# ZJU-FAST-Lab/uneven_planner

Measured on AMD Instinct MI355X. Metric: MINCO traj-opts/sec (batch), higher is better.
Workload: dtype f64

## Files before the change

### include/uneven_hip.h

```cpp
#ifndef UNEVEN_HIP_H
#define UNEVEN_HIP_H

#include <stdint.h>

#ifdef __cplusplus
extern "C" {
#endif

typedef struct uph_map uph_map;
typedef struct uph_ctx uph_ctx;
typedef struct uph_kino uph_kino;

#define UPH_OK 0
#define UPH_ERR_INVALID (-1)
#define UPH_ERR_HIP (-2)
#define UPH_ERR_NO_DEVICE (-3)
#define UPH_ERR_LIMIT (-4)
#define UPH_ERR_NO_CACHE (-5)

#define UPH_RET_STOPPED 3
#define UPH_RET_UNSUPPORTED 4

#define UPH_RET_LEFT_TILE 5
#define UPH_TILE_MARGIN 2.0
// ... 181 lines not shown
int uph_traj_states(uph_ctx* c, int32_t n, const int32_t* traj, const double* t, double* out10);
#define UPH_REFINE_AT_END 7
int uph_refine_upload(uph_ctx* src, uph_ctx* dst, int32_t B, const int32_t* src_traj, const double* t_switch, double* switch_states ,
                      int32_t* status, int32_t* traj_of, int32_t* n_inner_xy, int32_t* n_inner_yaw);
int uph_plan_staged(uph_ctx* c, int32_t cap_xy, int32_t cap_yaw, double* init_xy, double* end_xy, double* init_yaw, double* end_yaw, double* inner_xy,
                    double* inner_yaw, int32_t* n_inner_xy, int32_t* n_inner_yaw, double* total_time);

int uph_ctx_create(uph_map* m, const uph_opt_params* p, uph_ctx** out);
void uph_ctx_destroy(uph_ctx* c);
int uph_ctx_set_lanes(uph_ctx* c, int32_t lanes);
int uph_ctx_set_xcd_locality(uph_ctx* c, int32_t group);
int uph_ctx_set_wps(uph_ctx* c, int32_t wps);
int uph_ctx_set_sample_precision(uph_ctx* c, int32_t bits);
int uph_ctx_set_rho(uph_ctx* c, double rho);
int uph_ctx_get_rho(uph_ctx* c, double* rho);

int uph_ctx_set_trace(uph_ctx* c, int32_t cap);
int uph_ctx_get_trace(uph_ctx* c, double* out);

int uph_optimize_batch(uph_ctx* c, int32_t B, const uph_problem* probs, uph_result* results);
int uph_optimize_batch_multi(uph_ctx* const* ctxs, int32_t n_gpus, int32_t B, const uph_problem* probs, uph_result* results);
int uph_multi_batch_plan(int32_t n_gpus, int32_t B, const uph_problem* probs, int32_t* share_of, double* predicted_cost);
int uph_batch_count(const uph_ctx* c);
int uph_batch_origin(const uph_ctx* c, int32_t* idx);
int uph_batch_upload(uph_ctx* c, int32_t B, const uph_problem* probs);
int uph_batch_solve(uph_ctx* c);
int uph_batch_solve_async(uph_ctx* c);
int uph_batch_wait(uph_ctx* c);
int uph_batch_download(uph_ctx* c, uph_result* results);
int uph_batch_stats(uph_ctx* c, double* kernel_ms, int64_t* evals, int64_t* sample_evals, int64_t* lbfgs_iters, int64_t* hist_bytes);

int uph_batch_prepare_ms(uph_ctx* c, double* ms);

int uph_batch_cycles(uph_ctx* c, long long* out);

int uph_eval_batch(uph_ctx* c, const double* x_packed, double* f, double* grad_packed, int32_t repeat);
int uph_penalty_batch(uph_ctx* c, int32_t repeat, int32_t store_residuals, double* cost, double* gdcxy_packed, double* gdcyaw_packed, double* gdT2);
int uph_init_scaling_batch(uph_ctx* c);
int uph_microbench_batch(uph_ctx* c, int32_t reps);
int uph_batch_set_state(uph_ctx* c, const double* lambda, const double* mu, const double* scale_cx, const double* scale_fx, const double* rho);
int uph_batch_set_x(uph_ctx* c, const double* x_packed);
int uph_batch_alm_passes(uph_ctx* c, int32_t max_passes);
int uph_batch_set_lbfgs_state(uph_ctx* c, const double* g, const double* d, const double* pf, const double* lm_s, const double* lm_y, const double* lm_ys, const double* scal5);
int uph_batch_lbfgs_resume(uph_ctx* c, int32_t budget, int32_t finish_pass);
int uph_batch_get_lbfgs_state(uph_ctx* c, double* g, double* d, double* pf, double* lm_s, double* lm_y, double* lm_ys, double* scal8);
// ... 45 lines not shown
```

### uneven_planner_amd/_lib.py

```python
import ctypes as C
import os

_HERE = os.path.dirname(os.path.abspath(__file__))
LIB_PATH = os.environ.get("UNEVENHIP_LIB") or os.path.join(_HERE, "libunevenhip.so")


class MapParams(C.Structure):
    _fields_ = [("iter_num", C.c_int32), ("map_size_x", C.c_double), ("map_size_y", C.c_double),
                ("ellipsoid_x", C.c_double), ("ellipsoid_y", C.c_double), ("ellipsoid_z", C.c_double),
                ("xy_resolution", C.c_double), ("yaw_resolution", C.c_double), ("min_cnormal", C.c_double),
                ("max_rho", C.c_double), ("gravity", C.c_double)]


class OptParams(C.Structure):
    _fields_ = [("rho_T", C.c_double), ("rho_ter", C.c_double), ("max_vel", C.c_double), ("max_acc_lon", C.c_double),
                ("max_acc_lat", C.c_double), ("max_kap", C.c_double), ("min_cxi", C.c_double), ("max_sig", C.c_double),
                ("use_scaling", C.c_int32), ("rho", C.c_double), ("beta", C.c_double), ("gamma", C.c_double),
                ("epsilon_con", C.c_double), ("max_iter", C.c_double), ("g_epsilon", C.c_double),
                ("min_step", C.c_double), ("inner_max_iter", C.c_double), ("delta", C.c_double),
                ("mem_size", C.c_int32), ("past", C.c_int32), ("int_K", C.c_int32)]


class ManagerParams(C.Structure):
    _fields_ = [("piece_len", C.c_double), ("mean_vel", C.c_double), ("init_time_times", C.c_double), ("yaw_piece_times", C.c_double),
# ... 85 lines not shown
    "uph_frontend_query": (C.c_int, [_VP, DP, _I32, DP, C.POINTER(C.c_int32), C.POINTER(C.c_int32)]),
    "uph_terrain_pose_query": (C.c_int, [_VP, DP, _I32, DP]),
    "uph_frontend_query_ms": (C.c_int, [_VP, DP]),
    "uph_map_filter_cloud": (_I64, [C.POINTER(C.c_float), _I64, C.POINTER(C.c_float), _I64]),
    "uph_map_build_stats": (C.c_int, [_VP, DP, C.POINTER(_I64), C.POINTER(_I64)]),
    "uph_map_build_stages": (C.c_int, [_VP, DP]),
    "uph_map_built_cloud": (_I64, [_VP, C.POINTER(C.c_float), _I64]),
    "uph_ctx_create": (C.c_int, [_VP, C.POINTER(OptParams), C.POINTER(_VP)]),
    "uph_ctx_destroy": (None, [_VP]),
    "uph_ctx_set_lanes": (C.c_int, [_VP, _I32]),
    "uph_ctx_set_wps": (C.c_int, [_VP, _I32]),
    "uph_ctx_set_xcd_locality": (C.c_int, [_VP, _I32]),
    "uph_ctx_set_sample_precision": (C.c_int, [_VP, _I32]),
    "uph_ctx_set_rho": (C.c_int, [_VP, C.c_double]),
    "uph_ctx_get_rho": (C.c_int, [_VP, DP]),
    "uph_ctx_set_trace": (C.c_int, [_VP, _I32]),
    "uph_ctx_get_trace": (C.c_int, [_VP, DP]),
    "uph_optimize_batch": (C.c_int, [_VP, _I32, C.POINTER(Problem), C.POINTER(Result)]),
    "uph_batch_upload": (C.c_int, [_VP, _I32, C.POINTER(Problem)]),
    "uph_batch_solve": (C.c_int, [_VP]),
    "uph_batch_solve_async": (C.c_int, [_VP]),
    "uph_batch_wait": (C.c_int, [_VP]),
    "uph_batch_download": (C.c_int, [_VP, C.POINTER(Result)]),
    "uph_batch_stats": (C.c_int, [_VP, DP, C.POINTER(_I64), C.POINTER(_I64), C.POINTER(_I64), C.POINTER(_I64)]),
    "uph_batch_prepare_ms": (C.c_int, [_VP, DP]),
    "uph_batch_cycles": (C.c_int, [_VP, C.POINTER(C.c_longlong)]),
    "uph_build_id": (C.c_char_p, []),
    "uph_eval_batch": (C.c_int, [_VP, DP, DP, DP, _I32]),
    "uph_penalty_batch": (C.c_int, [_VP, _I32, _I32, DP, DP, DP, DP]),
    "uph_init_scaling_batch": (C.c_int, [_VP]),
    "uph_microbench_batch": (C.c_int, [_VP, _I32]),
    "uph_batch_set_state": (C.c_int, [_VP, DP, DP, DP, DP, DP]),
    "uph_report_batch": (C.c_int, [_VP, DP]),
    "uph_rollout_sizes": (C.c_int, [_I32, C.POINTER(_I32), DP, C.POINTER(_I32), DP, C.c_double, _I32, C.POINTER(_I64)]),
    "uph_rollout_plan": (C.c_int, [_VP, C.c_double, _I32, C.POINTER(_I64)]),
    "uph_rollout_batch": (C.c_int, [_VP, C.c_double, _I32, _I32, _I32, _I32, DP]),
    "uph_rollout_batch_dev": (C.c_int, [_VP, C.c_double, _I32, _I32, _I32, _I32, _VP]),
    "uph_batch_set_x": (C.c_int, [_VP, DP]),
    "uph_batch_alm_passes": (C.c_int, [_VP, _I32]),
    "uph_batch_set_lbfgs_state": (C.c_int, [_VP, DP, DP, DP, DP, DP, DP, DP]),
# ... 105 lines not shown
```

### uneven_planner_amd/alm_traj_opt.py

```python
import ctypes as C

import numpy as np

from . import _lib

HILL_OPT_PARAMS = dict(rho_T=100000.0, rho_ter=10.0, max_vel=0.5, max_acc_lon=5.0, max_acc_lat=10.0, max_kap=2.1,
                       min_cxi=0.8, max_sig=0.05, use_scaling=True, rho=1.0, beta=1000.0, gamma=1.0,
                       epsilon_con=0.001, max_iter=10.0, g_epsilon=1.0e-3, min_step=1.0e-32, inner_max_iter=10000.0,
                       delta=1.0e-4, mem_size=256, past=3, int_K=16)
_INT_FIELDS = ("use_scaling", "mem_size", "past", "int_K")


def pack_problems(probs, int_K=16, with_sizes=False):
    arr = (_lib.Problem * len(probs))()
    keep, sizes = [], []
    for i, pr in enumerate(probs):
        ixy = np.ascontiguousarray(np.asarray(pr["inner_xy"], dtype=np.float64).T)
        iyw = np.ascontiguousarray(pr["inner_yaw"], dtype=np.float64)
        keep += [ixy, iyw]
        a = arr[i]
        a.n_inner_xy, a.n_inner_yaw = ixy.shape[0], iyw.shape[0]
        a.init_xy[:] = np.asarray(pr["init_xy"], dtype=np.float64).T.ravel().tolist()
        a.end_xy[:] = np.asarray(pr["end_xy"], dtype=np.float64).T.ravel().tolist()
        a.init_yaw[:] = np.asarray(pr["init_yaw"], dtype=np.float64).ravel().tolist()
# ... 370 lines not shown
    def set_lanes(self, lanes):
        _lib.check(self.L.uph_ctx_set_lanes(self.h, int(lanes)), "uph_ctx_set_lanes")

    def set_xcd_locality(self, group):
        _lib.check(self.L.uph_ctx_set_xcd_locality(self.h, int(group)), "uph_ctx_set_xcd_locality")

    def set_wps(self, wps):
        _lib.check(self.L.uph_ctx_set_wps(self.h, int(wps)), "uph_ctx_set_wps")

    def set_sample_precision(self, bits):
        _lib.check(self.L.uph_ctx_set_sample_precision(self.h, int(bits)), "uph_ctx_set_sample_precision")

    def set_rho(self, rho):
        _lib.check(self.L.uph_ctx_set_rho(self.h, float(rho)), "uph_ctx_set_rho")

    def get_rho(self):
        r = C.c_double(0)
        _lib.check(self.L.uph_ctx_get_rho(self.h, C.byref(r)), "uph_ctx_get_rho")
        return r.value

    def _make_problems(self, probs):
        arr, keep, self._sizes = pack_problems(probs, int(self.int_K), with_sizes=True)
        return arr, keep

    def upload(self, probs):
        arr, keep = self._make_problems(probs)
        self._B = 0
        _lib.check(self.L.uph_batch_upload(self.h, len(probs), arr), "uph_batch_upload")
        self._B = len(probs)
        self._trace_cap_up = getattr(self, "_trace_cap", 0)
# ... 1 lines not shown
    def solve(self):
        _lib.check(self.L.uph_batch_solve(self.h), "uph_batch_solve")

    def solve_async(self):
        _lib.check(self.L.uph_batch_solve_async(self.h), "uph_batch_solve_async")

    def wait(self):
        _lib.check(self.L.uph_batch_wait(self.h), "uph_batch_wait")

    def stats(self):
        ms = C.c_double(0)
        v = [C.c_int64(0) for _ in range(4)]
        _lib.check(self.L.uph_batch_stats(self.h, C.byref(ms), *[C.byref(x) for x in v]), "uph_batch_stats")
        pm = C.c_double(0)
        _lib.check(self.L.uph_batch_prepare_ms(self.h, C.byref(pm)), "uph_batch_prepare_ms")
        return dict(kernel_ms=ms.value, prepare_ms=pm.value, evals=v[0].value, sample_evals=v[1].value, lbfgs_iters=v[2].value, hist_bytes=v[3].value)

    def cycles(self):
        out = np.zeros((max(0, self.L.uph_batch_count(self.h)), 16), dtype=np.int64)
        _lib.check(self.L.uph_batch_cycles(self.h, out.ctypes.data_as(C.POINTER(C.c_longlong))), "uph_batch_cycles")
        return out

    def origin(self):
        idx = np.zeros(max(0, self.L.uph_batch_count(self.h)), dtype=np.int32)
        _lib.check(self.L.uph_batch_origin(self.h, idx.ctypes.data_as(C.POINTER(C.c_int32))), "uph_batch_origin")
        return idx

    def download(self, full=True):
        res, bufs = self._result_array(self._sizes, full)
        _lib.check(self.L.uph_batch_download(self.h, res), "uph_batch_download")
        self._last = self._collect(res, bufs)
# ... 479 lines not shown
```

### uneven_planner_amd/csrc/solver_program.hpp

```cpp
#pragma once
#include "terrain_dev.hpp"
#include "trajectory_dev.hpp"
#include "uph_common.hpp"

namespace uph {

#ifndef UPH_GRID_FROM_MEM
#define UPH_GRID_FROM_MEM 1
#endif
#ifndef UPH_PHASE_MASK
#define UPH_PHASE_MASK 15
#endif
#ifndef UPH_SCALING_WB
#define UPH_SCALING_WB 8
#endif
#ifndef UPH_SC_XB
#define UPH_SC_XB 9
#endif
#ifndef UPH_SC_YB
#define UPH_SC_YB 14
#endif
#ifndef UPH_SC_WLO
#define UPH_SC_WLO 2
#endif
#ifndef UPH_SC_WHI
#define UPH_SC_WHI 3
#endif

template <class WG, class SR = double>
struct Solver {
    WG& wg;
    const GridDev& grid;
    const OptParams& P;
    const BatchDev& bd;
    const TrajDesc& td;
    int Nxy, Nyaw, n, S, K, mem, CH, CHP, recd;
    int CHS;
    int* rtag;
    double *x, *xp, *g, *gp, *d, *cxy, *cyaw, *Gxy, *Gyaw, *gamxy, *gamyaw, *bt, *rec, *wtab, *ttab, *pf, *hd;
    double *dual, *res, *scl, *hist;
    int hrow, hnp;
    const double *Wr_xy, *Wr_yaw;
    double rho, scale_fx, Txy, Tyaw, last_jerk, last_gd;
    long long hist_reads;
    long long cyc[16];
    long long t_last_eval_end;
    long long* sub_t = nullptr;
    int evals, bidx, trace_n;
    float inv_k1;
    double ec_irho, ec_step, ec_invK, ec_iTyaw, ec_omega, ec_omega_h;

    static constexpr int REC_FIELDS = 12;
    static UPH_HD size_t ldsDoubles(int Nxy, int Nyaw, int n, int CH, int mem, int K) {
        size_t recd = (size_t)REC_FIELDS * (CH + 1) + (CH + 1) / 2;
        const size_t nvec = 2 * (Nxy + 5) + (Nyaw + 5);
        const size_t knd = (size_t)knotBufDoubles(Nxy + 1, 4) + knotBufDoubles(Nyaw + 1, 2), adj = (size_t)knotBufDoubles(Nxy, 4) + knotBufDoubles(Nyaw, 2) + nvec;
        recd = recd < knd ? knd : recd;
        recd = recd < adj ? adj : recd;
        recd = recd < (size_t)mem ? (size_t)mem : recd;
        const size_t td_ = (size_t)Nxy + K + 2;
        return (size_t)5 * n + (nvec < td_ ? td_ : nvec) + 2 * (12 * Nxy + 6 * Nyaw) + recd + (size_t)6 * (K + 1) + THOMAS_DOUBLES + MAX_PAST + 8 + 18;
    }

    UPH_HD Solver(WG& w, const GridDev& gr, const OptParams& p, const BatchDev& b, int bi, double* lds)
        : wg(w), grid(gr), P(p), bd(b), td(b.desc[bi]) {
        bidx = bi;
        Nxy = td.Nxy; Nyaw = td.Nyaw; n = td.n; S = td.S; K = P.int_K; mem = P.mem_size;
        inv_k1 = 1.0f / (float)(K + 1);
        CH = wg.size(); CHP = CH + 1; recd = REC_FIELDS * CHP + (CH + 1) / 2;
        CHS = CH;
#if !defined(UPH_ALIGNED_CHUNKS) || UPH_ALIGNED_CHUNKS
        {
            const int ppc = CH / (K + 1);
            if (ppc >= 1 && (Nxy + ppc - 1) / ppc == (S + CH - 1) / CH) CHS = ppc * (K + 1);
        }
#endif
// ... 6 lines not shown
        q += nvec < Nxy + K + 2 ? Nxy + K + 2 : nvec;
        cxy = q; q += 12 * Nxy; cyaw = q; q += 6 * Nyaw;
        Gxy = q; q += 12 * Nxy; Gyaw = q; q += 6 * Nyaw;
        wtab = q; q += 6 * (K + 1);
        rec = q;
        {
            size_t rd = (size_t)recd;
            const size_t knd = (size_t)knotBufDoubles(Nxy + 1, 4) + knotBufDoubles(Nyaw + 1, 2), adj = (size_t)knotBufDoubles(Nxy, 4) + knotBufDoubles(Nyaw, 2) + nvec;
            rd = rd < knd ? knd : rd; rd = rd < adj ? adj : rd; rd = rd < (size_t)mem ? (size_t)mem : rd;
            q += rd;
        }
        rtag = (int*)(rec + (size_t)REC_FIELDS * CHP);
        ttab = q; q += THOMAS_DOUBLES;
        pf = q; q += MAX_PAST + 8;
        hd = q; q += 18;
        dual = bd.dual + 7 * td.off_s; res = bd.res + 7 * td.off_s; scl = bd.scl + 7 * td.off_s;
        hist = bd.hist + td.off_hist; hrow = histRowDoubles(n); hnp = 64 * histNQ(n);
        Wr_xy = bd.ops[td.op_xy].Wr; Wr_yaw = bd.ops[td.op_yaw].Wr;
        rho = 0; scale_fx = 1.0; Txy = Tyaw = 0; last_jerk = 0; hist_reads = 0; evals = 0; trace_n = 0;
        for (int q = 0; q < 16; q++) cyc[q] = 0;
        t_last_eval_end = 0;
        wg.pfor(18 + THOMAS_DOUBLES, [&](int t) {
            if (t < 18) hd[t] = t < 6 ? td.init_xy[t] : (t < 12 ? td.end_xy[t - 6] : (t < 15 ? td.init_yaw[t - 12] : td.end_yaw[t - 15]));
            else ttab[t - 18] = bd.thomas[t - 18];
        });
    }

    UPH_HD void tracePush(double v) {
        if (bd.trace != nullptr && trace_n < bd.trace_cap) {
            const int at = trace_n;
            wg.one([&]() { bd.trace[(size_t)bidx * bd.trace_cap + at] = v; });
        }
        trace_n++;
    }

    static UPH_HD int divSmall(int a, int b, float inv) {
        int q = (int)((float)a * inv);
// ... 584 lines not shown

    UPH_HD void evalConsts() {
        ec_irho = wg.bcast(1.0 / rho);
        ec_step = wg.bcast(Txy / K);
        ec_invK = wg.bcast(1.0 / K);
        ec_omega = wg.bcast(P.rho_ter * ec_step * scale_fx);
        ec_omega_h = wg.bcast(0.5 * P.rho_ter * ec_step * scale_fx);
    }

    UPH_HD void refreshResiduals() {
        UPH_MARK("refreshResiduals");
        wg.pfor(2, [&](int u) { fillTimes(u); });
        wg.pfor(S, [&](int s) { double dummy[3]; sampleEval<true>(s, 0, dummy); });
    }

    template <bool STEP>
    UPH_HD double eval(double* xin, double* gout, double st = 0.0) {
        evals++;
        long long t0 = wg.clock();
        if (t_last_eval_end) cyc[5] += t0 - t_last_eval_end;
        if (UPH_PHASE_MASK & 1) generate<STEP>(xin, st);
        const double tau = wg.bcast(xin[0]);
        const double jw = wg.bcast(P.use_scaling ? scale_trick_jerk * scale_fx : scale_fx);
        double js[3] = {0.0, 0.0, 0.0};
        if (UPH_PHASE_MASK & 1) expand(xin, jw, js);
        long long t1 = wg.clock(); cyc[0] += t1 - t0;
        last_jerk = js[0];
        const double jerk_cost = wg.bcast(P.use_scaling ? js[0] * scale_fx * scale_trick_jerk : js[0] * scale_fx);
        evalConsts();
        double sm[3] = {0.0, 0.0, 0.0};
        wg.template accBegin<3>();
        for (int s0 = 0; s0 < S; s0 += CHS) {
            const int cnt = S - s0 < CHS ? S - s0 : CHS;
            t0 = wg.clock();
            if (UPH_PHASE_MASK & 2) wg.template accChunk<3>(cnt, [&](int t, double* acc) { sampleEval<false, SR>(s0 + t, t, acc); });
            t1 = wg.clock(); cyc[1] += t1 - t0;
            if (UPH_PHASE_MASK & 4) scatterChunk(s0, cnt);
            cyc[2] += wg.clock() - t1;
        }
        wg.template accEnd<3>(sm);
        t1 = wg.clock();
        double chx = 0.0, chy = 0.0, gdw = 0.0;
        if (UPH_PHASE_MASK & 8) adjoint(chx, chy, gout, &gdw);
        t0 = wg.clock(); cyc[3] += t0 - t1;
        const double gTx = js[1] * jw + sm[1] + chx;
        const double gTy = js[2] * jw + sm[2] + chy;
        const double grad_Tsum = P.rho_T * scale_fx + gTx / Nxy + gTy / Nyaw;
        const double g0 = wg.bcast(grad_Tsum * getTtoTauGrad(tau));
        wg.pfor(1, [&](int) { gout[0] = g0; });
        last_gd = wg.bcast(gdw + g0 * d[0]);
        const double tau_cost = P.rho_T * expC2(tau) * scale_fx;
        t_last_eval_end = wg.clock();
        return wg.bcast(jerk_cost + sm[0] + tau_cost);
    }

    UPH_HD void initScaling(double* x0) {
// ... 211 lines not shown
                double headtail_y = 0.0;
                headtail_y += a0[0] * hd[13];
                headtail_y += 2.0 * Ty * a0[1] * hd[14];
                headtail_y += a0[2] * hd[16];
                headtail_y += 2.0 * Ty * a0[3] * hd[17];
                hty[q] = headtail_y;
            }
        }
#pragma unroll
        for (int q = 0; q < NQS; q++) {
            const double gTau = ((sumx[q] + htx[q]) / Nxy + (sumy[q] + hty[q]) / Nyaw) * dTau;
            scl[(Q0 + q) * S + s] = 1.0 / dmax(1.0, dmax(mx[q], fabs(gTau)));
        }
    }

    UPH_HD int lineSearch(double& f, double& stp, double stpmin, double stpmax, double dginit) {
        int count = 0;
        bool brackt = false, touched = false;
        double mu = 0.0, nu = stpmax;
        if (!(stp > 0.0)) return LBFGSERR_INVALIDPARAMETERS;
        if (0.0 < dginit) return LBFGSERR_INCREASEGRADIENT;
        const double finit = wg.bcast(f);
        const double dgtest = wg.bcast(P.f_dec_coeff * dginit);
        const double dstest = wg.bcast(P.s_curv_coeff * dginit);
        while (true) {
            f = eval<true>(x, g, stp);
            ++count;
            if (isinf(f) || isnan(f)) return LBFGSERR_INVALID_FUNCVAL;
            if (P.past > 0 && fabs(finit - f) / (fabs(finit) + 1.0) < P.delta / P.past) return count;
            if (f > finit + stp * dgtest) {
                nu = stp;
                brackt = true;
            } else {
                if (last_gd < dstest) mu = stp;
                else return count;
            }
            if (P.max_linesearch <= count) return LBFGSERR_MAXIMUMLINESEARCH;
            if (brackt && (nu - mu) < P.machine_prec * nu) return LBFGSERR_WIDTHTOOSMALL;
            if (brackt) stp = wg.bcast(0.5 * (mu + nu));
            else stp = wg.bcast(stp * 2.0);
            if (stp < stpmin) return LBFGSERR_MINIMUMSTEP;
            if (stp > stpmax) {
                if (touched) return LBFGSERR_MAXIMUMSTEP;
                touched = true;
                stp = stpmax;
// ... 90 lines not shown
                    wg.twoLoop(d, g, n, hist, pf + MAX_PAST, rec, m, end, bound, ys / yy);
                    dginit = wg.bcast(pf[MAX_PAST]);
                    t_last_eval_end = wg.clock();
                    cyc[4] += t_last_eval_end - tq;
                    hist_reads += (long long)4 * bound * n;
                }
                step = 1.0;
            }
        }
        if constexpr (RESUME) { io->step = step; io->fx = fx; io->k = k; io->end = end; io->bound = bound; }
        f_out = fx;
        k_out = k;
        return ret;
    }

    UPH_HD void updateDualVars() {
        UPH_MARK("updateDualVars");
        const double r = rho;
        wg.pfor(S, [&](int s) {
            dual[s] += r * res[s];
            for (int q = 1; q < 7; q++) dual[q * S + s] = dmax(dual[q * S + s] + r * res[q * S + s], 0.0);
        });
        rho = wg.bcast(dmin((1 + P.gamma) * rho, P.beta));
    }
    UPH_HD bool judgeConvergence() {
        const double r = rho;
        const double rh = wg.maxv(S, [&](int s) { return fabs(res[s]); });
        const double rg = wg.maxv(6 * S, [&](int t) { return fabs(dmax(res[S + t], -dual[S + t] / r)); });
        return dmax(rh, rg) < P.epsilon_con;
    }

    UPH_HD void storeTrajectory(TrajState& st) {
        double* oc = bd.cxy + td.off_cxy;
        double* oy = bd.cyaw + td.off_cyaw;
        wg.pfor(12 * Nxy + 6 * Nyaw, [&](int t) { if (t < 12 * Nxy) oc[t] = cxy[t]; else oy[t - 12 * Nxy] = cyaw[t - 12 * Nxy]; });
        wg.pfor(1, [&](int) {
            st.T_xy = Txy; st.T_yaw = Tyaw; st.jerk_cost = last_jerk; st.scale_fx = scale_fx; st.rho = rho;
            st.evals = evals; st.hist_reads = hist_reads;
#ifdef UPH_TL_PROF
            for (int q = 0; q < 6; q++) cyc[8 + q] = wg.tl[q];
#endif
            for (int q = 0; q < 16; q++) st.cyc[q] = cyc[q];
        });
#ifdef UPH_BAR_PROF
        wg.sync();
        wg.dumpBar(&st.cyc[8]);
#endif
    }

    UPH_HD void prepare(TrajState& st) {
        const double* gx0 = bd.x0 + td.off_x;
        double* gx = bd.x + td.off_x;
        rho = wg.bcast(st.rho);
        scale_fx = 1.0;
        wg.pfor(S > n ? S : n, [&](int t) {
            if (t < n) { x[t] = gx0[t]; gx[t] = gx0[t]; }
            if (t < S) for (int q = 0; q < 7; q++) { dual[q * S + t] = 0.0; res[q * S + t] = 0.0; scl[q * S + t] = 1.0; }
        });
        const long long tstart = wg.clock();
        if (P.use_scaling) initScaling(x);
        cyc[5] += wg.clock() - tstart;
        wg.pfor(1, [&](int) { st.scale_fx = scale_fx; st.cyc[5] = cyc[5]; });
    }

    UPH_HD void optimize(TrajState& st, int cap = 0) {
        double* gx0 = bd.x + td.off_x;
        rho = wg.bcast(st.rho);
        scale_fx = wg.bcast(st.scale_fx);
        wg.pfor(n, [&](int t) { x[t] = gx0[t]; });
        const long long tstart = wg.clock();
        cyc[14] = wg.realtime();
        int ret_code = 0, iter = 0, total_k = 0, last_ret = 0;
        double inner_cost = 0.0;
        while (true) {
            int kk = 0;
            tracePush(-1.0);
            const int result = lbfgs<false>(inner_cost, kk);
            refreshResiduals();
            total_k += kk;
            last_ret = result;
            if (result == LBFGS_CONVERGENCE || result == LBFGS_CANCELED || result == LBFGS_STOP || result == LBFGSERR_MAXIMUMITERATION) {
            } else if (result == LBFGSERR_MAXIMUMLINESEARCH) {
            } else { ret_code = 1; break; }
            updateDualVars();
// ... 4 lines not shown
        wg.pfor(n, [&](int t) { gx0[t] = x[t]; bd.gout[td.off_x + t] = g[t]; });
        cyc[6] = wg.clock() - tstart;
        cyc[15] = wg.realtime();
        storeTrajectory(st);
        wg.pfor(1, [&](int) {
            st.ret_code = ret_code; st.alm_iters = iter; st.lbfgs_iters = total_k; st.last_lbfgs_ret = last_ret; st.f = inner_cost;
        });
    }

    UPH_HD void resumeHook(TrajState& st, int budget, int finish) {
        double* gx = bd.x + td.off_x;
        double* gg = bd.gout + td.off_x;
        double* gd = bd.rs_d + td.off_x;
        double* rs = bd.rs + (size_t)bidx * 24;
        rho = wg.bcast(st.rho); scale_fx = wg.bcast(st.scale_fx);
        wg.pfor(n + MAX_PAST, [&](int t) { if (t < n) { x[t] = gx[t]; g[t] = gg[t]; d[t] = gd[t]; } else pf[t - n] = rs[8 + t - n]; });
        ResumeIO io;
        io.step = wg.bcast(rs[0]); io.fx = wg.bcast(rs[1]);
        io.k = (int)wg.bcast(rs[2]); io.end = (int)wg.bcast(rs[3]); io.bound = (int)wg.bcast(rs[4]); io.budget = budget;
        double f = 0.0;
        int kk = 0;
        const int ret = lbfgs<true>(f, kk, &io);
        int accepted = 0, conv = 0;
        if (evals > 0) refreshResiduals();
        if (finish && ret != LBFGS_RUNNING_HOOK) {
            accepted = (ret == LBFGS_CONVERGENCE || ret == LBFGS_CANCELED || ret == LBFGS_STOP || ret == LBFGSERR_MAXIMUMITERATION || ret == LBFGSERR_MAXIMUMLINESEARCH) ? 1 : 0;
            if (accepted) { updateDualVars(); conv = judgeConvergence() ? 1 : 0; }
        }
        wg.pfor(n + MAX_PAST, [&](int t) { if (t < n) { gx[t] = x[t]; gg[t] = g[t]; gd[t] = d[t]; } else rs[8 + t - n] = pf[t - n]; });
        wg.pfor(1, [&](int) {
// ... 158 lines not shown
```

### uneven_planner_amd/csrc/unevenhip.hip

```cpp
#include <hip/hip_runtime.h>

#include <type_traits>

#include <algorithm>
#include <cmath>
#include <cstdio>
#include <cstdlib>
#include <cstring>
#include <map>
#include <numeric>
#include <string>
#include <thread>
#include <vector>

#include "../../include/uneven_hip.h"
#include "minco_op_host.hpp"
#include "resample_walk.hpp"
#include "solver_program.hpp"
#include "uph_ctx.hpp"
#include "wave_dev.hpp"

using namespace uph;

#ifndef UPH_THOMAS_KPL
// ... 836 lines not shown
    if (p->mem_size < 1 || p->mem_size > UPH_MAX_MEM || p->past < 0 || p->past > UPH_MAX_PAST || p->int_K < 1 || p->int_K > 64) {
        setError("uph_ctx_create: mem_size/past/int_K outside compiled limits");
        return UPH_ERR_LIMIT;
    }
    HIPCHK(hipSetDevice(uphMapDevice(m)));
    uph_ctx* c = new uph_ctx();
    c->map = m;
    c->device = uphMapDevice(m);
    OptParams& P = c->P;
    P.rho_T = p->rho_T; P.rho_ter = p->rho_ter; P.max_vel = p->max_vel; P.max_acc_lon = p->max_acc_lon; P.max_acc_lat = p->max_acc_lat;
    P.max_kap = p->max_kap; P.min_cxi = p->min_cxi; P.max_sig = p->max_sig; P.use_scaling = p->use_scaling;
    P.beta = p->beta; P.gamma = p->gamma; P.epsilon_con = p->epsilon_con; P.max_iter = p->max_iter;
    P.g_epsilon = p->g_epsilon; P.min_step = p->min_step; P.delta = p->delta;
    P.inner_max_iter = (int)p->inner_max_iter; P.mem_size = p->mem_size; P.past = p->past; P.int_K = p->int_K;
    P.max_linesearch = 64; P.max_step = 1.0e20; P.f_dec_coeff = 1.0e-4; P.s_curv_coeff = 0.9; P.cautious_factor = 1.0e-6; P.machine_prec = 1.0e-16;
    finishParams(P);
    c->rho = p->rho;
    {
        std::vector<double> tab;
        buildThomasTable(tab);
        if (c->d_thomas.ensure(tab.size() * sizeof(double))) { delete c; return UPH_ERR_HIP; }
        if (hipMemcpy(c->d_thomas.p, tab.data(), tab.size() * sizeof(double), hipMemcpyHostToDevice) != hipSuccess) { setError("hipMemcpy(thomas table) failed"); c->d_thomas.release(); delete c; return UPH_ERR_HIP; }
    }
    HIPCHK(hipStreamCreateWithFlags(&c->stream, hipStreamNonBlocking));
    {
        int prio_lo = 0, prio_hi = 0;
        hipDeviceGetStreamPriorityRange(&prio_lo, &prio_hi);
        HIPCHK(hipStreamCreateWithPriority(&c->stream2, hipStreamNonBlocking, prio_hi));
    }
    HIPCHK(hipEventCreate(&c->ev2));
// ... 27 lines not shown
}

int uph_ctx_set_lanes(uph_ctx* c, int32_t lanes) {
    if (!c || (lanes != 0 && lanes != 64 && lanes != 128 && lanes != 256 && lanes != 512)) return UPH_ERR_INVALID;
    c->lanes_forced = lanes;
    return UPH_OK;
}
int uph_ctx_set_xcd_locality(uph_ctx* c, int32_t group) { if (!c || group < 0) return UPH_ERR_INVALID; c->xcd_group = group; return UPH_OK; }
int uph_ctx_set_wps(uph_ctx* c, int32_t wps) { if (!c || wps < 0 || wps > 2) return UPH_ERR_INVALID; c->wps_forced = wps; return UPH_OK; }
int uph_ctx_set_sample_precision(uph_ctx* c, int32_t bits) {
    if (!c || (bits != 32 && bits != 64)) { setError("uph_ctx_set_sample_precision: 32 or 64"); return UPH_ERR_INVALID; }
    c->sample_f32 = bits == 32;
    return UPH_OK;
}
int uph_ctx_set_rho(uph_ctx* c, double rho) { if (!c) return UPH_ERR_INVALID; c->rho = rho; return UPH_OK; }
int uph_ctx_get_rho(uph_ctx* c, double* rho) { if (!c || !rho) return UPH_ERR_INVALID; *rho = c->rho; return UPH_OK; }

int uph_ctx_set_trace(uph_ctx* c, int32_t cap) { if (!c || cap < 0) return UPH_ERR_INVALID; c->trace_cap = cap; return UPH_OK; }
int uph_ctx_get_trace(uph_ctx* c, double* out ) {
    if (c && c->pending) { setError("an asynchronous solve is in flight on this context: call uph_batch_wait first"); return UPH_ERR_INVALID; }
    if (!c || !out || c->trace_cap_up <= 0 || c->B <= 0) return UPH_ERR_INVALID;
    HIPCHK(hipSetDevice(uphMapDevice(c->map)));
    HIPCHK(hipMemcpy(out, c->d_trace.p, sizeof(double) * (size_t)c->B * c->trace_cap_up, hipMemcpyDeviceToHost));
    return UPH_OK;
}

static void yawTurnKink(const uph_problem& pr, double& turn, double& kink) {
    double prev = pr.init_yaw[0];
    turn = 0.0; kink = 0.0;
    for (int i = 0; i <= pr.n_inner_yaw; i++) {
// ... 500 lines not shown
}

int uph_batch_wait(uph_ctx* c) {
    if (!c || !c->pending) { setError("uph_batch_wait: no asynchronous solve in flight"); return UPH_ERR_INVALID; }
    HIPCHK(hipSetDevice(uphMapDevice(c->map)));
    c->pending = false;
    HIPCHK(hipStreamSynchronize(c->stream));
    float ms = 0.f;
    HIPCHK(hipEventElapsedTime(&ms, c->evp0, c->evp1));
    c->last_prepare_ms = ms;
    HIPCHK(hipEventElapsedTime(&ms, c->ev0, c->ev1));
    c->last_ms = ms;
    int r = refreshStates(c);
    if (r != UPH_OK) return r;
    c->last_evals = c->last_sample_evals = c->last_iters = c->last_hist_bytes = 0;
    for (int b = 0; b < c->B; b++) {
        if (c->rejected[b]) continue;
        const TrajState& s = c->state_host[b];
        c->last_evals += s.evals;
        c->last_sample_evals += (int64_t)s.evals * c->desc[b].S;
        c->last_iters += s.lbfgs_iters;
        c->last_hist_bytes += s.hist_reads * 8;
    }
    if (c->B == 1 && !c->rejected[0]) c->rho = c->state_host[0].rho;
    return UPH_OK;
}

int uph_batch_solve(uph_ctx* c) {
    const int r = uph_batch_solve_async(c);
    return r != UPH_OK ? r : uph_batch_wait(c);
}

int uph_batch_count(const uph_ctx* c) { return c ? c->B : UPH_ERR_INVALID; }
int uph_batch_origin(const uph_ctx* c, int32_t* idx) {
    if (!c || !idx || c->B <= 0) { setError("uph_batch_origin: no batch uploaded"); return UPH_ERR_INVALID; }
    for (int b = 0; b < c->B; b++) idx[b] = c->origin.empty() ? b : c->origin[b];
    return UPH_OK;
}

int uph_batch_stats(uph_ctx* c, double* kernel_ms, int64_t* evals, int64_t* sample_evals, int64_t* lbfgs_iters, int64_t* hist_bytes) {
    if (!c) return UPH_ERR_INVALID;
    if (kernel_ms) *kernel_ms = c->last_ms;
    if (evals) *evals = c->last_evals;
    if (sample_evals) *sample_evals = c->last_sample_evals;
    if (lbfgs_iters) *lbfgs_iters = c->last_iters;
    if (hist_bytes) *hist_bytes = c->last_hist_bytes;
    return UPH_OK;
}

int uph_batch_prepare_ms(uph_ctx* c, double* ms) { if (!c || !ms) return UPH_ERR_INVALID; *ms = c->last_prepare_ms; return UPH_OK; }

int uph_batch_cycles(uph_ctx* c, long long* out) {
    if (!c || c->B <= 0 || !out) return UPH_ERR_INVALID;
    for (int b = 0; b < c->B; b++) for (int q = 0; q < 16; q++) out[b * 16 + q] = c->state_host[b].cyc[q];
    return UPH_OK;
}

int uph_batch_download(uph_ctx* c, uph_result* results) {
    if (!c || c->B <= 0 || !results) { setError("uph_batch_download: bad arguments"); return UPH_ERR_INVALID; }
    if (c->pending) { setError("uph_batch_download: an asynchronous solve is in flight (uph_batch_wait first)"); return UPH_ERR_INVALID; }
    HIPCHK(hipSetDevice(uphMapDevice(c->map)));
// ... 231 lines not shown
    int r = launchSolver(c, 4, 1);
    if (r != UPH_OK) return r;
    return refreshStates(c);
}

int uph_report_batch(uph_ctx* c, double* out7) {
    if (!c || c->B <= 0 || !out7) { setError("uph_report_batch: bad arguments"); return UPH_ERR_INVALID; }
    int r = launchSolver(c, 3, 1);
    if (r != UPH_OK) return r;
    HIPCHK(hipMemcpy(out7, c->d_report.p, 8 * 7 * c->B, hipMemcpyDeviceToHost));
    return UPH_OK;
}

static void collectSolveStats(uph_ctx* c) {
    c->last_evals = c->last_sample_evals = c->last_iters = c->last_hist_bytes = 0;
    for (int b = 0; b < c->B; b++) {
        if (c->rejected[b]) continue;
        const TrajState& s = c->state_host[b];
        c->last_evals += s.evals;
        c->last_sample_evals += (int64_t)s.evals * c->desc[b].S;
        c->last_iters += s.lbfgs_iters;
        c->last_hist_bytes += s.hist_reads * 8;
    }
}
int uph_batch_set_x(uph_ctx* c, const double* x_packed) {
    if (c && c->pending) { setError("an asynchronous solve is in flight on this context: call uph_batch_wait first"); return UPH_ERR_INVALID; }
    if (c && c->n_rejected) { setError("packed-array hooks need a batch without unsupported problems (uph_result.ret_code == UPH_RET_UNSUPPORTED)"); return UPH_ERR_INVALID; }
    if (!c || c->B <= 0 || !x_packed) { setError("uph_batch_set_x: bad arguments"); return UPH_ERR_INVALID; }
    HIPCHK(hipSetDevice(c->device));
    return uploadPackedX(c, x_packed);
}
int uph_batch_alm_passes(uph_ctx* c, int32_t max_passes) {
    if (!c || c->B <= 0 || max_passes < 0) { setError("uph_batch_alm_passes: bad arguments"); return UPH_ERR_INVALID; }
    int r = launchSolver(c, 2, max_passes);
    if (r != UPH_OK) return r;
// ... 89 lines not shown
```

### uneven_planner_amd/csrc/uph_common.hpp

```cpp
#pragma once
#include <math.h>
#include <stdint.h>

#if defined(__HIPCC__)
#define UPH_HD __host__ __device__ __forceinline__
#define UPH_NOINLINE __host__ __device__ __attribute__((noinline))
#else
#define UPH_HD inline
#define UPH_NOINLINE __attribute__((noinline))
#endif

#if defined(__HIP_DEVICE_COMPILE__)
#define UPH_AS_GLOBAL(p) ((const __attribute__((address_space(1))) double*)(p))
#else
#define UPH_AS_GLOBAL(p) (p)
#endif

#if defined(UPH_ISA_MARKS) && defined(__HIP_DEVICE_COMPILE__)
#define UPH_MARK(name) asm volatile("; UPHMARK " name)
#else
#define UPH_MARK(name) do { } while (0)
#endif

namespace uph {
// ... 44 lines not shown
    double half_xy, half_yaw;
    double gravity;
    const double* cells;
    const float* cells32;
};

struct OptParams {
    double rho_T, rho_ter, max_vel, max_acc_lon, max_acc_lat, max_kap, min_cxi, max_sig;
    int use_scaling;
    double beta, gamma, epsilon_con, max_iter;
    double g_epsilon, min_step, delta;
    int inner_max_iter, mem_size, past, int_K;
    int max_linesearch;
    double max_step, f_dec_coeff, s_curv_coeff, cautious_factor, machine_prec;
    double max_vel2, max_acc_lon2, max_acc_lat2, max_kap2;
};

inline void finishGrid(GridDev& g) {
    for (int i = 0; i < 3; i++) { g.lo[i] = g.minb[i] + 1e-4; g.hi[i] = g.maxb[i] - 1e-4; }
    g.half_xy = 0.5 * g.xy_res; g.half_yaw = 0.5 * g.yaw_res;
}
inline void finishParams(OptParams& P) {
    P.max_vel2 = P.max_vel * P.max_vel; P.max_acc_lon2 = P.max_acc_lon * P.max_acc_lon;
    P.max_acc_lat2 = P.max_acc_lat * P.max_acc_lat; P.max_kap2 = P.max_kap * P.max_kap;
}

struct MincoOp {
    int N;
    const double* Wt;
    const double* Wr;
// ... 16 lines not shown
    int Nxy, Nyaw, n, S;
    int op_xy, op_yaw;
    int64_t off_x;
    int64_t off_s;
    int64_t off_cxy, off_cyaw;
    int64_t off_hist;
    double init_xy[6], end_xy[6], init_yaw[3], end_yaw[3];
};

struct TrajState {
    double rho, scale_fx;
    double f, jerk_cost, T_xy, T_yaw;
    int ret_code, alm_iters, lbfgs_iters, evals, last_lbfgs_ret, pad;
    long long hist_reads;
    long long cyc[16];
};

struct BatchDev {
    int B;
    const TrajDesc* desc;
    TrajState* state;
    const MincoOp* ops;
    const double* x0;
    double* x;
    double* gout;
    double* dual;
    double* res;
    double* scl;
    double* cxy;
    double* cyaw;
// ... 179 lines not shown
```

### uneven_planner_amd/csrc/uph_ctx.hpp

```cpp
#pragma once
#include <hip/hip_runtime.h>

#include <map>
#include <string>
#include <vector>

#include "uph_internal.hpp"

using namespace uph;

struct DevBuf {
    void* p = nullptr;
    size_t cap = 0;
    int ensure(size_t bytes) {
        if (bytes <= cap) return 0;
        if (p) hipFree(p);
        p = nullptr; cap = 0;
        size_t want = bytes + bytes / 4 + 256;
        if (hipMalloc(&p, want) != hipSuccess) { setError("hipMalloc failed"); return -1; }
        cap = want;
        return 0;
    }
    void release() { if (p) hipFree(p); p = nullptr; cap = 0; }
    template <class T> T* as() { return (T*)p; }
// ... 73 lines not shown
    std::vector<ProblemHead> plan_probs;
    std::vector<double> end_pose;
    std::vector<double> end_bnd;
    DevBuf d_sw_q, d_sw_out;
    DevBuf d_refine_rec;
    DevBuf d_win_q, d_win_out;
    double last_check_ms = 0.0;
    double last_locate_ms = 0.0;
    double last_sep_ms = 0.0;
    int trace_cap = 0;
    int trace_cap_up = 0;
    std::vector<TrajState> state_host;
    HostBuf h_x, h_cxy, h_cyaw, h_dual, h_res, h_scl;
    double last_ms = 0.0, last_prepare_ms = 0.0;
    int64_t last_evals = 0, last_sample_evals = 0, last_iters = 0, last_hist_bytes = 0;
};

#define HIPCHK(call)                                                                               \
    do {                                                                                           \
        hipError_t _e = (call);                                                                    \
        if (_e != hipSuccess) {                                                                    \
            setError(std::string(#call) + ": " + hipGetErrorString(_e));                           \
            return UPH_ERR_HIP;                                                                    \
        }                                                                                          \
    } while (0)

int refreshStates(uph_ctx* c);
int syncGridMem(uph_ctx* c, uph::GridDev& grid);

struct SwitchQuery {
// ... 9 lines not shown
```

Baseline: 50200.

## Abandon line-search trial evaluations early when a lower bound exceeds the Armijo threshold

During the line search, each trial evaluation gets a rejection threshold. Before sampling, a lower bound built from jerk cost, time cost and a dual-norm bound (maintained after each dual update) is compared to it, so trials that must fail the sufficient-decrease test skip sampling and the adjoint. After sampling, a second check skips the adjoint and gradient when the trial already exceeds the threshold. Abandoning only happens when the search would continue, and it adds per-trial broadcasts, a dual-norm reduction and counters. The risk is that the bound or tolerances alter which trials pass, changing trajectories.

```diff
diff --git a/include/uneven_hip.h b/include/uneven_hip.h
--- a/include/uneven_hip.h
+++ b/include/uneven_hip.h
@@ -219,6 +219,7 @@
 int uph_ctx_set_sample_precision(uph_ctx* c, int32_t bits);
 int uph_ctx_set_rho(uph_ctx* c, double rho);
 int uph_ctx_get_rho(uph_ctx* c, double* rho);
+int uph_ctx_set_trial_abandon(uph_ctx* c, int32_t on);
 
 int uph_ctx_set_trace(uph_ctx* c, int32_t cap);
 int uph_ctx_get_trace(uph_ctx* c, double* out);
@@ -234,6 +235,7 @@
 int uph_batch_wait(uph_ctx* c);
 int uph_batch_download(uph_ctx* c, uph_result* results);
 int uph_batch_stats(uph_ctx* c, double* kernel_ms, int64_t* evals, int64_t* sample_evals, int64_t* lbfgs_iters, int64_t* hist_bytes);
+int uph_batch_abandon_stats(uph_ctx* c, int64_t* out5);
 
 int uph_batch_prepare_ms(uph_ctx* c, double* ms);
 
diff --git a/uneven_planner_amd/_lib.py b/uneven_planner_amd/_lib.py
--- a/uneven_planner_amd/_lib.py
+++ b/uneven_planner_amd/_lib.py
@@ -123,6 +123,7 @@
     "uph_ctx_set_sample_precision": (C.c_int, [_VP, _I32]),
     "uph_ctx_set_rho": (C.c_int, [_VP, C.c_double]),
     "uph_ctx_get_rho": (C.c_int, [_VP, DP]),
+    "uph_ctx_set_trial_abandon": (C.c_int, [_VP, _I32]),
     "uph_ctx_set_trace": (C.c_int, [_VP, _I32]),
     "uph_ctx_get_trace": (C.c_int, [_VP, DP]),
     "uph_optimize_batch": (C.c_int, [_VP, _I32, C.POINTER(Problem), C.POINTER(Result)]),
@@ -133,6 +134,7 @@
     "uph_batch_download": (C.c_int, [_VP, C.POINTER(Result)]),
     "uph_batch_stats": (C.c_int, [_VP, DP, C.POINTER(_I64), C.POINTER(_I64), C.POINTER(_I64), C.POINTER(_I64)]),
     "uph_batch_prepare_ms": (C.c_int, [_VP, DP]),
+    "uph_batch_abandon_stats": (C.c_int, [_VP, C.POINTER(_I64)]),
     "uph_batch_cycles": (C.c_int, [_VP, C.POINTER(C.c_longlong)]),
     "uph_build_id": (C.c_char_p, []),
     "uph_eval_batch": (C.c_int, [_VP, DP, DP, DP, _I32]),
diff --git a/uneven_planner_amd/alm_traj_opt.py b/uneven_planner_amd/alm_traj_opt.py
--- a/uneven_planner_amd/alm_traj_opt.py
+++ b/uneven_planner_amd/alm_traj_opt.py
@@ -408,6 +408,9 @@
     def set_rho(self, rho):
         _lib.check(self.L.uph_ctx_set_rho(self.h, float(rho)), "uph_ctx_set_rho")
 
+    def set_trial_abandon(self, on):
+        _lib.check(self.L.uph_ctx_set_trial_abandon(self.h, 1 if on else 0), "uph_ctx_set_trial_abandon")
+
     def get_rho(self):
         r = C.c_double(0)
         _lib.check(self.L.uph_ctx_get_rho(self.h, C.byref(r)), "uph_ctx_get_rho")
@@ -439,7 +442,10 @@
         _lib.check(self.L.uph_batch_stats(self.h, C.byref(ms), *[C.byref(x) for x in v]), "uph_batch_stats")
         pm = C.c_double(0)
         _lib.check(self.L.uph_batch_prepare_ms(self.h, C.byref(pm)), "uph_batch_prepare_ms")
-        return dict(kernel_ms=ms.value, prepare_ms=pm.value, evals=v[0].value, sample_evals=v[1].value, lbfgs_iters=v[2].value, hist_bytes=v[3].value)
+        ab = (C.c_int64 * 5)()
+        _lib.check(self.L.uph_batch_abandon_stats(self.h, ab), "uph_batch_abandon_stats")
+        return dict(kernel_ms=ms.value, prepare_ms=pm.value, evals=v[0].value, sample_evals=v[1].value, lbfgs_iters=v[2].value, hist_bytes=v[3].value,
+                    ls_rejected=ab[0], ls_guarded=ab[1], ls_abandoned=ab[2], chunks_skipped=ab[3], adjoints_skipped=ab[4])
 
     def cycles(self):
         out = np.zeros((max(0, self.L.uph_batch_count(self.h)), 16), dtype=np.int64)
diff --git a/uneven_planner_amd/csrc/solver_program.hpp b/uneven_planner_amd/csrc/solver_program.hpp
--- a/uneven_planner_amd/csrc/solver_program.hpp
+++ b/uneven_planner_amd/csrc/solver_program.hpp
@@ -10,6 +10,9 @@
 #endif
 #ifndef UPH_PHASE_MASK
 #define UPH_PHASE_MASK 15
+#endif
+#ifndef UPH_STATE_PROBE
+#define UPH_STATE_PROBE(st) do { } while (0)
 #endif
 #ifndef UPH_SCALING_WB
 #define UPH_SCALING_WB 8
@@ -38,6 +41,16 @@
     int CHS;
     int* rtag;
     double *x, *xp, *g, *gp, *d, *cxy, *cyaw, *Gxy, *Gyaw, *gamxy, *gamyaw, *bt, *rec, *wtab, *ttab, *pf, *hd;
+    double* ab;
+    int* abn;
+    static constexpr int AB_DOUBLES = 4;
+    UPH_HD void tally(int k, bool yes) {
+#if defined(__HIP_DEVICE_COMPILE__)
+        if (yes && wg.wave == 0) abn[k] = abn[k] + 1;
+#else
+        if (yes) abn[k]++;
+#endif
+    }
     double *dual, *res, *scl, *hist;
     int hrow, hnp;
     const double *Wr_xy, *Wr_yaw;
@@ -59,7 +72,7 @@
         recd = recd < adj ? adj : recd;
         recd = recd < (size_t)mem ? (size_t)mem : recd;
         const size_t td_ = (size_t)Nxy + K + 2;
-        return (size_t)5 * n + (nvec < td_ ? td_ : nvec) + 2 * (12 * Nxy + 6 * Nyaw) + recd + (size_t)6 * (K + 1) + THOMAS_DOUBLES + MAX_PAST + 8 + 18;
+        return (size_t)5 * n + (nvec < td_ ? td_ : nvec) + 2 * (12 * Nxy + 6 * Nyaw) + recd + (size_t)6 * (K + 1) + THOMAS_DOUBLES + MAX_PAST + 8 + 18 + AB_DOUBLES;
     }
 
     UPH_HD Solver(WG& w, const GridDev& gr, const OptParams& p, const BatchDev& b, int bi, double* lds)
@@ -96,6 +109,8 @@
         ttab = q; q += THOMAS_DOUBLES;
         pf = q; q += MAX_PAST + 8;
         hd = q; q += 18;
+        ab = q; q += AB_DOUBLES;
+        abn = (int*)(ab + 1);
         dual = bd.dual + 7 * td.off_s; res = bd.res + 7 * td.off_s; scl = bd.scl + 7 * td.off_s;
         hist = bd.hist + td.off_hist; hrow = histRowDoubles(n); hnp = 64 * histNQ(n);
         Wr_xy = bd.ops[td.op_xy].Wr; Wr_yaw = bd.ops[td.op_yaw].Wr;
@@ -103,6 +118,7 @@
         for (int q = 0; q < 16; q++) cyc[q] = 0;
         t_last_eval_end = 0;
         wg.pfor(18 + THOMAS_DOUBLES, [&](int t) {
+            if (t == 0) { ab[0] = 0.0; abn[0] = abn[1] = abn[2] = abn[3] = 0; }
             if (t < 18) hd[t] = t < 6 ? td.init_xy[t] : (t < 12 ? td.end_xy[t - 6] : (t < 15 ? td.init_yaw[t - 12] : td.end_yaw[t - 15]));
             else ttab[t - 18] = bd.thomas[t - 18];
         });
@@ -717,8 +733,9 @@
         wg.pfor(S, [&](int s) { double dummy[3]; sampleEval<true>(s, 0, dummy); });
     }
 
+    static constexpr double ABANDON_REL = 1e-9, ABANDON_REL_F = 1e-14;
     template <bool STEP>
-    UPH_HD double eval(double* xin, double* gout, double st = 0.0) {
+    UPH_HD double eval(double* xin, double* gout, double st = 0.0, double thr = __builtin_huge_val()) {
         evals++;
         long long t0 = wg.clock();
         if (t_last_eval_end) cyc[5] += t0 - t_last_eval_end;
@@ -731,6 +748,19 @@
         last_jerk = js[0];
         const double jerk_cost = wg.bcast(P.use_scaling ? js[0] * scale_fx * scale_trick_jerk : js[0] * scale_fx);
         evalConsts();
+        if (STEP && thr < __builtin_huge_val()) {
+            double tq = tau;
+            pinv(tq);
+            const double tau_lb = P.rho_T * expC2(tq) * scale_fx;
+            const double lbd = wg.bcast(ab[0]);
+            const double L0 = wg.bcast(jerk_cost + tau_lb - lbd);
+            const double mag = wg.bcast(fabs(jerk_cost) + fabs(tau_lb) + lbd);
+            if (L0 > thr + ABANDON_REL * mag && L0 < __builtin_huge_val() && ec_omega >= 0.0) {
+                tally(2, true);
+                t_last_eval_end = wg.clock();
+                return L0;
+            }
+        }
         double sm[3] = {0.0, 0.0, 0.0};
         wg.template accBegin<3>();
         for (int s0 = 0; s0 < S; s0 += CHS) {
@@ -743,6 +773,18 @@
         }
         wg.template accEnd<3>(sm);
         t1 = wg.clock();
+        if (STEP && thr < __builtin_huge_val()) {
+            double tq = tau;
+            pinv(tq);
+            const double tau_q = P.rho_T * expC2(tq) * scale_fx;
+            const double fq = wg.bcast(jerk_cost + sm[0] + tau_q);
+            const double mag = wg.bcast(fabs(jerk_cost) + fabs(sm[0]) + fabs(tau_q));
+            if (fq > thr + ABANDON_REL_F * mag && fq < __builtin_huge_val()) {
+                tally(3, true);
+                t_last_eval_end = wg.clock();
+                return fq;
+            }
+        }
         double chx = 0.0, chy = 0.0, gdw = 0.0;
         if (UPH_PHASE_MASK & 8) adjoint(chx, chy, gout, &gdw);
         t0 = wg.clock(); cyc[3] += t0 - t1;
@@ -984,6 +1026,20 @@
         }
     }
 
+    UPH_HD bool abandonAllowed() const {
+        if (sizeof(SR) != sizeof(double)) return false;
+#if defined(__HIP_DEVICE_COMPILE__) && UPH_GRID_FROM_MEM
+        typedef const __attribute__((address_space(4))) int* pi_t;
+        pi_t pt = (pi_t)(const void*)&bd.params_mem->no_trial_abandon;
+        asm volatile("" : "+s"(pt));
+        return *pt == 0;
+#else
+        return P.no_trial_abandon == 0;
+#endif
+    }
+    static UPH_HD bool noExitAfterRejection(int count, double stp, double mu, double stpmin, double stpmax, int max_linesearch, double machine_prec) {
+        return count + 1 < max_linesearch && (stp - mu) >= machine_prec * stp && 0.5 * (mu + stp) >= stpmin && stp <= stpmax;
+    }
     UPH_HD int lineSearch(double& f, double& stp, double stpmin, double stpmax, double dginit) {
         int count = 0;
         bool brackt = false, touched = false;
@@ -993,12 +1049,18 @@
         const double finit = wg.bcast(f);
         const double dgtest = wg.bcast(P.f_dec_coeff * dginit);
         const double dstest = wg.bcast(P.s_curv_coeff * dginit);
+        const bool on = abandonAllowed();
+        const double pst = wg.bcast(P.past > 0 ? P.delta / P.past * (fabs(finit) + 1.0) : 0.0);
         while (true) {
-            f = eval<true>(x, g, stp);
+            const double arm = stp * dgtest;
+            const bool may = on && noExitAfterRejection(count, stp, mu, stpmin, stpmax, P.max_linesearch, P.machine_prec);
+            const double thr = wg.bcast(may ? dmax(finit + arm, finit + pst) + ABANDON_REL * (fabs(finit) + fabs(arm) + pst) : __builtin_huge_val());
+            f = eval<true>(x, g, stp, thr);
             ++count;
             if (isinf(f) || isnan(f)) return LBFGSERR_INVALID_FUNCVAL;
             if (P.past > 0 && fabs(finit - f) / (fabs(finit) + 1.0) < P.delta / P.past) return count;
             if (f > finit + stp * dgtest) {
+                tally(0, on); tally(1, on && !may);
                 nu = stp;
                 brackt = true;
             } else {
@@ -1119,14 +1181,32 @@
         return ret;
     }
 
+    UPH_HD void setDualBound(double sq) {
+        const double v = rho > 0.0 ? sq * (0.5 / rho) : __builtin_huge_val();
+        wg.one([&]() { ab[0] = v; });
+    }
+    UPH_HD void formDualBound() {
+        double sq[1];
+        wg.template sum<1>(S, sq, [&](int s, double* acc) {
+            double a = 0.0;
+            for (int q = 0; q < 7; q++) { const double v = dual[q * S + s]; a += v * v; }
+            acc[0] += a;
+        });
+        setDualBound(sq[0]);
+    }
     UPH_HD void updateDualVars() {
         UPH_MARK("updateDualVars");
         const double r = rho;
-        wg.pfor(S, [&](int s) {
+        double sq[1];
+        wg.template sum<1>(S, sq, [&](int s, double* acc) {
             dual[s] += r * res[s];
             for (int q = 1; q < 7; q++) dual[q * S + s] = dmax(dual[q * S + s] + r * res[q * S + s], 0.0);
+            double a = 0.0;
+            for (int q = 0; q < 7; q++) { const double v = dual[q * S + s]; a += v * v; }
+            acc[0] += a;
         });
         rho = wg.bcast(dmin((1 + P.gamma) * rho, P.beta));
+        setDualBound(sq[0]);
     }
     UPH_HD bool judgeConvergence() {
         const double r = rho;
@@ -1142,11 +1222,14 @@
         wg.pfor(1, [&](int) {
             st.T_xy = Txy; st.T_yaw = Tyaw; st.jerk_cost = last_jerk; st.scale_fx = scale_fx; st.rho = rho;
             st.evals = evals; st.hist_reads = hist_reads;
+            st.ls_rejected = abn[0]; st.ls_guarded = abn[1]; st.ls_abandoned = abn[2]; st.adjoints_skipped = abn[3] + abn[2];
+            st.chunks_skipped = abn[2] * ((S + CHS - 1) / CHS);
 #ifdef UPH_TL_PROF
             for (int q = 0; q < 6; q++) cyc[8 + q] = wg.tl[q];
 #endif
             for (int q = 0; q < 16; q++) st.cyc[q] = cyc[q];
         });
+        UPH_STATE_PROBE(st);
 #ifdef UPH_BAR_PROF
         wg.sync();
         wg.dumpBar(&st.cyc[8]);
@@ -1173,6 +1256,7 @@
         rho = wg.bcast(st.rho);
         scale_fx = wg.bcast(st.scale_fx);
         wg.pfor(n, [&](int t) { x[t] = gx0[t]; });
+        formDualBound();
         const long long tstart = wg.clock();
         cyc[14] = wg.realtime();
         int ret_code = 0, iter = 0, total_k = 0, last_ret = 0;
@@ -1207,6 +1291,7 @@
         double* gd = bd.rs_d + td.off_x;
         double* rs = bd.rs + (size_t)bidx * 24;
         rho = wg.bcast(st.rho); scale_fx = wg.bcast(st.scale_fx);
+        formDualBound();
         wg.pfor(n + MAX_PAST, [&](int t) { if (t < n) { x[t] = gx[t]; g[t] = gg[t]; d[t] = gd[t]; } else pf[t - n] = rs[8 + t - n]; });
         ResumeIO io;
         io.step = wg.bcast(rs[0]); io.fx = wg.bcast(rs[1]);
diff --git a/uneven_planner_amd/csrc/unevenhip.hip b/uneven_planner_amd/csrc/unevenhip.hip
--- a/uneven_planner_amd/csrc/unevenhip.hip
+++ b/uneven_planner_amd/csrc/unevenhip.hip
@@ -874,6 +874,7 @@
     P.g_epsilon = p->g_epsilon; P.min_step = p->min_step; P.delta = p->delta;
     P.inner_max_iter = (int)p->inner_max_iter; P.mem_size = p->mem_size; P.past = p->past; P.int_K = p->int_K;
     P.max_linesearch = 64; P.max_step = 1.0e20; P.f_dec_coeff = 1.0e-4; P.s_curv_coeff = 0.9; P.cautious_factor = 1.0e-6; P.machine_prec = 1.0e-16;
+    P.no_trial_abandon = 0; P.pad_ = 0;
     finishParams(P);
     c->rho = p->rho;
     {
@@ -931,6 +932,7 @@
     return UPH_OK;
 }
 int uph_ctx_set_rho(uph_ctx* c, double rho) { if (!c) return UPH_ERR_INVALID; c->rho = rho; return UPH_OK; }
+int uph_ctx_set_trial_abandon(uph_ctx* c, int32_t on) { if (!c || (on != 0 && on != 1)) return UPH_ERR_INVALID; c->P.no_trial_abandon = on ? 0 : 1; return UPH_OK; }
 int uph_ctx_get_rho(uph_ctx* c, double* rho) { if (!c || !rho) return UPH_ERR_INVALID; *rho = c->rho; return UPH_OK; }
 
 int uph_ctx_set_trace(uph_ctx* c, int32_t cap) { if (!c || cap < 0) return UPH_ERR_INVALID; c->trace_cap = cap; return UPH_OK; }
@@ -1461,11 +1463,14 @@
     int r = refreshStates(c);
     if (r != UPH_OK) return r;
     c->last_evals = c->last_sample_evals = c->last_iters = c->last_hist_bytes = 0;
+    for (int q = 0; q < 5; q++) c->last_abandon[q] = 0;
     for (int b = 0; b < c->B; b++) {
         if (c->rejected[b]) continue;
         const TrajState& s = c->state_host[b];
         c->last_evals += s.evals;
-        c->last_sample_evals += (int64_t)s.evals * c->desc[b].S;
+        c->last_sample_evals += (int64_t)(s.evals - s.ls_abandoned) * c->desc[b].S;
+        c->last_abandon[0] += s.ls_rejected; c->last_abandon[1] += s.ls_guarded; c->last_abandon[2] += s.ls_abandoned;
+        c->last_abandon[3] += s.chunks_skipped; c->last_abandon[4] += s.adjoints_skipped;
         c->last_iters += s.lbfgs_iters;
         c->last_hist_bytes += s.hist_reads * 8;
     }
@@ -1492,6 +1497,12 @@
     if (sample_evals) *sample_evals = c->last_sample_evals;
     if (lbfgs_iters) *lbfgs_iters = c->last_iters;
     if (hist_bytes) *hist_bytes = c->last_hist_bytes;
+    return UPH_OK;
+}
+
+int uph_batch_abandon_stats(uph_ctx* c, int64_t* out5) {
+    if (!c || !out5) return UPH_ERR_INVALID;
+    for (int q = 0; q < 5; q++) out5[q] = c->last_abandon[q];
     return UPH_OK;
 }
 
@@ -1753,11 +1764,14 @@
 
 static void collectSolveStats(uph_ctx* c) {
     c->last_evals = c->last_sample_evals = c->last_iters = c->last_hist_bytes = 0;
+    for (int q = 0; q < 5; q++) c->last_abandon[q] = 0;
     for (int b = 0; b < c->B; b++) {
         if (c->rejected[b]) continue;
         const TrajState& s = c->state_host[b];
         c->last_evals += s.evals;
-        c->last_sample_evals += (int64_t)s.evals * c->desc[b].S;
+        c->last_sample_evals += (int64_t)(s.evals - s.ls_abandoned) * c->desc[b].S;
+        c->last_abandon[0] += s.ls_rejected; c->last_abandon[1] += s.ls_guarded; c->last_abandon[2] += s.ls_abandoned;
+        c->last_abandon[3] += s.chunks_skipped; c->last_abandon[4] += s.adjoints_skipped;
         c->last_iters += s.lbfgs_iters;
         c->last_hist_bytes += s.hist_reads * 8;
     }
diff --git a/uneven_planner_amd/csrc/uph_common.hpp b/uneven_planner_amd/csrc/uph_common.hpp
--- a/uneven_planner_amd/csrc/uph_common.hpp
+++ b/uneven_planner_amd/csrc/uph_common.hpp
@@ -82,6 +82,7 @@
     int max_linesearch;
     double max_step, f_dec_coeff, s_curv_coeff, cautious_factor, machine_prec;
     double max_vel2, max_acc_lon2, max_acc_lat2, max_kap2;
+    int no_trial_abandon = 0, pad_ = 0;
 };
 
 inline void finishGrid(GridDev& g) {
@@ -128,6 +129,7 @@
     int ret_code, alm_iters, lbfgs_iters, evals, last_lbfgs_ret, pad;
     long long hist_reads;
     long long cyc[16];
+    int ls_rejected, ls_guarded, ls_abandoned, chunks_skipped, adjoints_skipped, pad2;
 };
 
 struct BatchDev {
diff --git a/uneven_planner_amd/csrc/uph_ctx.hpp b/uneven_planner_amd/csrc/uph_ctx.hpp
--- a/uneven_planner_amd/csrc/uph_ctx.hpp
+++ b/uneven_planner_amd/csrc/uph_ctx.hpp
@@ -111,6 +111,7 @@
     HostBuf h_x, h_cxy, h_cyaw, h_dual, h_res, h_scl;
     double last_ms = 0.0, last_prepare_ms = 0.0;
     int64_t last_evals = 0, last_sample_evals = 0, last_iters = 0, last_hist_bytes = 0;
+    int64_t last_abandon[5] = {0, 0, 0, 0, 0};
 };
 
 #define HIPCHK(call)                                                                               \
```

Result: faster. 53160, median of 6 (+5.9%).
